# abhisrkckl/PulsePortraiture

Hardware: AMD Instinct MI355X
Metric: subint portrait fits/sec (phase+DM, 512ch×2048bin) at 1/2/4/8 MI355X (higher is better)
Workload: dtype f64

## Files before the change

### pulseportraiture_amd/csrc/ppf_wfft2.hpp

```cpp
#pragma once
#include "ppf_wfft.hpp"

namespace ppf {
namespace wf2 {

#define WF2_CUT() __builtin_amdgcn_sched_barrier(0)

constexpr int kN = 1024;
constexpr int kXS = 65;
constexpr int kXSlots = 16 * kXS;
constexpr int kSpSlots = 32;

struct Seeds {
    double2 w1;
    double2 v1;
};

__device__ __forceinline__ Seeds make_seeds(int lane) {
    Seeds s;
    double sn, cs;
    sincospi(-2.0 * (double)lane / 1024.0, &sn, &cs);
    s.w1 = cmk(cs, sn);
    sincospi(-2.0 * (double)(lane & 15) / 64.0, &sn, &cs);
    s.v1 = cmk(cs, sn);
// ... 47 lines not shown
        const double p = fma(-T[e], b.y, b.x), q = fma(T[e], b.x, b.y);
        u = cmk(fma(C[e], p, a.x), fma(C[e], q, a.y));
        v = cmk(fma(-C[e], p, a.x), fma(-C[e], q, a.y));
    }
}
template <int LEN, int I, int J>
__device__ __forceinline__ void dft16_bfly(double2 (&y)[16]) {
    if constexpr (J < LEN / 2) {
        bfly16<J * (16 / LEN)>(y[I + J], y[I + J + LEN / 2]);
        dft16_bfly<LEN, I, J + 1>(y);
    }
}
template <int LEN, int I>
__device__ __forceinline__ void dft16_group(double2 (&y)[16]) {
    if constexpr (I < 16) {
        dft16_bfly<LEN, I, 0>(y);
        dft16_group<LEN, I + LEN>(y);
    }
}
__device__ __forceinline__ void dft16(double2 (&x)[16]) {
    double2 y[16];
    wfft::dft_perm<16, 0>(x, y);
    dft16_group<2, 0>(y);
    dft16_group<4, 0>(y);
    dft16_group<8, 0>(y);
    dft16_group<16, 0>(y);
#pragma unroll
    for (int i = 0; i < 16; ++i) x[i] = y[i];
}

__device__ __forceinline__ void opaque(double2 &v) {
    asm volatile("" : "+v"(v.x), "+v"(v.y));
}
__device__ __forceinline__ void fft1024(double2 (&x)[16], double2 *xb, int lane, const Seeds &sd0) {
    Seeds sd = sd0;
    opaque(sd.w1);
    opaque(sd.v1);
    dft16(x);
    {
        double2 wq = sd.w1;
        x[1] = cmul(x[1], wq);
#pragma unroll
        for (int k = 2; k < 16; ++k) {
            wq = cmul(wq, sd.w1);
            x[k] = cmul(x[k], wq);
        }
    }
    WF2_CUT();
#pragma unroll
    for (int r = 0; r < 8; ++r) pswap<true>(x[r], x[r + 8]);
#pragma unroll
    for (int r = 0; r < 16; ++r)
        if ((r & 4) == 0) pswap<false>(x[r], x[r + 4]);
    const double2 v2 = cmul(sd.v1, sd.v1);
#pragma unroll
    for (int a = 0; a < 4; ++a) {
        double2 t[4] = {x[a], x[a + 4], x[a + 8], x[a + 12]};
        wfft::dft<4>(t);
        x[a] = t[0];
        x[a + 4] = cmul(t[1], sd.v1);
        x[a + 8] = cmulc(t[2], v2);
        x[a + 12] = cmulc(t[3], sd.v1);
    }
    WF2_CUT();
    const int llo = lane & 15, k1hi = lane >> 4;
    const int lb0 = kXS * llo + 4 * k1hi;
    const int lb1 = kXS * ((16 - llo) & 15) - 4 * k1hi + 32;
    const int lb8 = lb1 + (k1hi == 0 ? 0 : 32);
#pragma unroll
    for (int a = 0; a < 4; ++a) {
        xb[lb0 + a] = x[a];
        xb[lb0 + a + 16] = x[a + 4];
        if (a == 0) xb[lb8] = x[8];
        else xb[lb1 + 32 - a] = x[a + 8];
        xb[lb1 + 16 - a] = x[a + 12];
    }
    wfft::wave_sync();
#pragma unroll
    for (int r = 0; r < 16; ++r) x[r] = xb[lane + kXS * r];
    wfft::wave_sync();
    dft16(x);
}

__device__ __forceinline__ int lane_kappa(int lane) {
    return lane < 32 ? lane : (lane == 32 ? 32 : 96 - lane);
}
__device__ __forceinline__ int out_index(int lane, int m) {
    const int kap = lane_kappa(lane);
    return lane < 32 ? kap + 64 * m : kap + 64 * (15 - m);
}

__device__ __forceinline__ int pair_k0(int lane) {
    return lane == 32 ? 32 : (lane & 31) + (lane >= 32 ? 512 : 0);
}
__device__ __forceinline__ void pairs(double2 (&x)[16], double2 *sp, int lane, double2 &zm) {
    const bool special = (lane & 31) == 0;
    if (special) {
        const int b = (lane >> 5) * 16;
#pragma unroll
        for (int m = 0; m < 16; ++m) sp[b + m] = x[m];
    }
#pragma unroll
    for (int i = 0; i < 8; ++i) pswap<true>(x[i], x[i + 8]);
    wfft::wave_sync();
    if (special) {
        const bool l0 = lane == 0;
#pragma unroll
        for (int i = 0; i < 8; ++i) {
            x[i] = sp[l0 ? i : 31 - i];
            x[i + 8] = sp[l0 ? ((16 - i) & 15) : 16 + i];
        }
        if (l0) zm = sp[8];
    }
    wfft::wave_sync();
}

}
}
```

### pulseportraiture_amd/csrc/ppf_xspec.hip

```cpp
#include <cstdlib>
#include <cstring>
#include <type_traits>

#include "ppf_internal.hpp"
#include "ppf_state.hpp"
#include "ppf_wfft.hpp"
#include "ppf_wfft2.hpp"

namespace ppf {

constexpr int kXW = 8;
template <int LOG2N>
__host__ __device__ constexpr int xsw() { return LOG2N == 10 ? 4 : 8; }
typedef double f64x4 __attribute__((ext_vector_type(4)));
typedef float vf2 __attribute__((ext_vector_type(2)));
typedef double vd2 __attribute__((ext_vector_type(2)));
typedef float vf4 __attribute__((ext_vector_type(4)));
#define SCHED_CUT() __builtin_amdgcn_sched_barrier(0)

__device__ __forceinline__ void block_map(int xcd_swizzle, int nblk, int &s, int &cb, int nsub = 0) {
    if (xcd_swizzle == 2) {
        const int per = nblk / 8, x = blockIdx.x % 8, r = blockIdx.x / 8;
        cb = x * per + r / nsub;
        s = r % nsub;
// ... 514 lines not shown
            const double u = (double)(k - N / 2) * ih;
            const double v = u * u, v2 = v * v, v4 = v2 * v2, v8 = v4 * v4;
            const double bv = ((bj & 1) ? v : 1.0) * ((bj & 2) ? v2 : 1.0) * ((bj & 4) ? v4 : 1.0) *
                              ((bj & 8) ? v8 : 1.0);
            d0 = __builtin_amdgcn_mfma_f64_16x16x4f64(abase[2 * se], bv, d0, 0, 0, 0);
            d1 = __builtin_amdgcn_mfma_f64_16x16x4f64(abase[2 * so], bv, d1, 0, 0, 0);
        }
        XP(4);
        const int om = (tid >> 1) & 31, ori = tid & 1;
        double val = 0.0;
        if (om == 0) val = reinterpret_cast<const double *>(buf + SIDE)[ori];
        const double ie = reinterpret_cast<const double *>(buf + SIDE2)[0];
        __syncthreads();
        {
            double *sc = reinterpret_cast<double *>(buf);
#pragma unroll
            for (int rr = 0; rr < 4; ++rr) {
                sc[rr * 64 + lane] = d0[rr];
                sc[256 + rr * 64 + lane] = d1[rr];
            }
        }
        __syncthreads();
        {
            const int row = 2 * wave + ori;
            const int idx = (om & 1) * 256 + (row >> 2) * 64 + ((row & 3) << 4) + (om >> 1);
#pragma unroll
            for (int w2 = 0; w2 < XW; ++w2) val += reinterpret_cast<const double *>(lds + w2 * SLW)[idx];
            unsigned mo = (unsigned)(om * 2 + ori);
            asm volatile("" : "+v"(mo));
            if (live) mom[(int64_t)n * kMoments * 2 + mo] = val * ie;
        }
        __syncthreads();
        XP(5);
    }
    XP_DONE();
}

__global__ void k_btab(int N, double *Bt) {
    const int i = blockIdx.x * blockDim.x + threadIdx.x;
    if (i >= N / 2 * 16) return;
    const int k = i >> 4, j = i & 15;
    const double u = (double)(k - N / 2) * (2.0 / (double)N);
    const double v = u * u, v2 = v * v, v4 = v2 * v2, v8 = v4 * v4;
    Bt[i] = ((j & 1) ? v : 1.0) * ((j & 2) ? v2 : 1.0) * ((j & 4) ? v4 : 1.0) * ((j & 8) ? v8 : 1.0);
}

__global__ void k_model_pow(const double2 *Mft, int nrows, int nharm, double *out) {
    const int lane = threadIdx.x & 63;
    const int row = blockIdx.x * (blockDim.x >> 6) + (threadIdx.x >> 6);
    if (row >= nrows) return;
    const double2 *M = Mft + (int64_t)row * nharm;
    double acc = 0.0;
    for (int k = lane + 1; k < nharm; k += 64) acc += cabs2(M[k]);
    acc = wave_sum(acc);
    if (lane == 0) out[row] = acc;
}

__global__ __launch_bounds__(256) void k_model_sum(const double2 *Mft, int nchan, int nharm,
                                                   int nmodel, double2 *out) {
    __shared__ double2 part[16][17];
    const int kl = threadIdx.x & 15, grp = threadIdx.x >> 4;
    const int k = blockIdx.x * 16 + kl;
    const int m = blockIdx.y;
    const int per = (nchan + 15) / 16;
    const int n0 = grp * per, n1 = min(nchan, n0 + per);
    double2 acc = cmk(0.0, 0.0);
    if (k < nharm) {
        const double2 *M = Mft + (int64_t)m * nchan * nharm + k;
#pragma unroll 8
        for (int n = n0; n < n1; ++n) acc = cadd(acc, M[(int64_t)n * nharm]);
    }
    part[grp][kl] = acc;
    __syncthreads();
    if (grp == 0 && k < nharm) {
        double2 t = part[0][kl];
        for (int g = 1; g < 16; ++g) t = cadd(t, part[g][kl]);
        out[(int64_t)m * nharm + k] = t;
    }
}

constexpr int kX2W = 4;
constexpr int kX2SL = wf2::kXSlots + wf2::kSpSlots;
constexpr int kX2IE = 1041;
__device__ __forceinline__ int x2slot(int k) { return k + (k >> 6); }

template <int DT, bool GS, bool TL>
__device__ __forceinline__ void xspec_w2_block(const XspecArgs &a, const int s, const int cb) {
    constexpr int N = 1024, NH = N + 1;
    constexpr bool GR = TL;
    constexpr bool LT = GR && GS;
    constexpr int MD = 4;
    using RowT = typename std::conditional<DT == 0, vf2, vd2>::type;
    extern __shared__ __attribute__((aligned(16))) double2 lds[];
    const int lane0 = threadIdx.x & 63;
    const int wave = __builtin_amdgcn_readfirstlane(threadIdx.x >> 6);
    double2 *buf = lds + wave * kX2SL;

    const int cbase = cb * a.cb, cend = min(a.nchan, cbase + a.cb);
    const int nround = (cend - cbase + kX2W - 1) / kX2W;
    const RowT *rows = reinterpret_cast<const RowT *>(a.data);
    RowT zr[16];
    auto fetch = [&](int n) {
        const RowT *src = rows + ((int64_t)s * a.nchan + n) * N;
#pragma unroll
        for (int q = 0; q < 16; ++q) zr[q] = __builtin_nontemporal_load(src + lane0 + 64 * q);
    };
    auto fetch_c = [&](int m) { fetch(m < cend ? m : cend - 1); };
    auto rows_ready = [&]() {
#pragma unroll
        for (int q = 0; q < 16; ++q) asm volatile("" ::"v"(zr[q].x), "v"(zr[q].y));
    };
    int n = cbase + wave;
    if constexpr (TL) fetch_c(n);
    const int cls = a.cls[s];
    const int mi = a.model_index ? a.model_index[s] : 0;
    const int xsl = a.xslot ? a.xslot[s] : s;
    double g_Dg = 0.0, g_nrm2 = 0.0, g_w2e2 = 0.0;
    if constexpr (GS) {
        g_Dg = readfirst_d(a.rec[(int64_t)s * kRecN + kRecDg]);
        g_nrm2 = readfirst_d(a.rec[(int64_t)s * kRecN + kRecNuRefM2]);
    }
    if (a.needx && !(cls & kClsNeedX)) return;
    if (((cls & kClsTile) != 0) != TL) return;
    const bool gon = GS && (cls & kClsGflag) != 0;
    const uint8_t *mask = a.mask ? a.mask + (int64_t)s * a.nchan : nullptr;
    const int nl = cbase + lane0;
    const bool lin = nl < cend;
    const int nlc = lin ? nl : cend - 1;
    const int64_t scn = (int64_t)s * a.nchan + nlc;
    const int nkw = (cbase & ~63) + lane0;
    int ld_kc = a.KC ? a.KC[(int64_t)mi * a.nchan + (nkw < a.nchan ? nkw : a.nchan - 1)] : 0;
    int ld_mask = mask ? mask[nlc] : 1;
    double ld_mpow = a.Mpow[(int64_t)mi * a.nchan + nlc];
    double ld_err = a.errs ? a.errs[scn] : 0.0;
    double ld_wn = 0.0, ld_f = 1.0;
    if constexpr (GS) {
        ld_wn = a.guess_weights[scn];
        ld_f = a.freqs[scn];
    }
    const double sqrtN = sqrt((double)N);
    const wf2::Seeds sd = wf2::make_seeds(lane0);
    double2 wA0, wstep;
    {
        double sn, cs;
        sincospi(-(double)wf2::pair_k0(lane0) / (double)N, &sn, &cs);
        wA0 = cmk(cs, sn);
        sincospi(-64.0 / (double)N, &sn, &cs);
        wstep = cmk(cs, sn);
    }
    asm volatile("" : "+v"(ld_kc), "+v"(ld_mask), "+v"(ld_mpow), "+v"(ld_err), "+v"(ld_wn), "+v"(ld_f));
    double2 *Xs = a.X + (int64_t)xsl * a.xnh * a.nchan;
    int kw = NH;
    if (a.KC) kw = (int)wave_max(nkw < a.nchan ? (double)ld_kc : 1.0);
    auto store_tiles = [&](int n, const double2 *b, double ie2, bool ok) {
        const int kwp = (kw + kXTile - 1) & ~(kXTile - 1);
        double2 *Xn = Xs + (int64_t)n * kXTile + (lane0 & (kXTile - 1));
#pragma unroll 1
        for (int h = lane0; h < kwp; h += 64) {
            const double2 v = (ok && h < kw) ? cscale(b[x2slot(h)], ie2) : cmk(0.0, 0.0);
            __builtin_nontemporal_store(vd2{v.x, v.y},
                                        reinterpret_cast<vd2 *>(Xn + (int64_t)(h >> 3) * a.nchan * kXTile));
        }
    };
    const int mlane = (lin && ld_mask) ? 1 : 0;
    auto usable = [&](int n) {
        return n < cend && __builtin_amdgcn_readlane(mlane, n - cbase) != 0;
    };
    constexpr int NL = 64 * guess_npl(10);
    double2 *gacc = lds + kX2W * kX2SL;
    if constexpr (GS && !GR) {
        if (gon) {
            for (int t = threadIdx.x; t < NL; t += 64 * kX2W) gacc[t] = cmk(0.0, 0.0);
            __syncthreads();
        }
    }
    double2 gr[8];
#pragma unroll
    for (int i = 0; i < 8; ++i) gr[i] = cmk(0.0, 0.0);
    const double ch_mpow = lin ? ld_mpow : 0.0;
    const double ch_err = (a.errs && lin) ? ld_err : 0.0;
    double ch_wn = 0.0, ch_dg = 0.0;
    if (GS && gon && lin) {
        ch_wn = ld_wn;
        ch_dg = g_Dg * (1.0 / (ld_f * ld_f) - g_nrm2);
    }
    double2 ch_e1 = cmk(1.0, 0.0);
    if constexpr (GR) {
        if (GS && gon) ch_e1 = cexp2pi(ch_dg);
    }
    double2 *ltab = lds + kX2W * kX2SL;
    if constexpr (LT) {
        if (wave == 0) {
            ltab[lane0] = sd.w1;
            ltab[64 + lane0] = sd.v1;
            ltab[128 + lane0] = wA0;
            ltab[192 + lane0] = ch_e1;
        }
        __syncthreads();
    }
    if constexpr (!TL) fetch_c(n);
    rows_ready();
    XP_INIT();
    for (int r = 0; r < nround; ++r, n += kX2W) {
        const bool live = usable(n);
        if (n < cend && !live && lane0 < 4) a.chan[((int64_t)s * a.nchan + n) * 4 + lane0] = 0.0;
        double2 x[16];
#pragma unroll
        for (int q = 0; q < 16; ++q) {
            x[q] = cmk((double)zr[q].x, (double)zr[q].y);
            asm volatile("" : "+v"(x[q].x), "+v"(x[q].y));
        }
        int lane = lane0;
        asm volatile("" : "+v"(lane));
        const bool lo = lane <= 32;
        const int kA = wf2::pair_k0(lane);
        const int hl0 = lo ? kA : N - kA, hstep = lo ? 64 : -64;
        const double2 *Mrow = a.Mft + ((int64_t)mi * a.nchan + (n < cend ? n : cend - 1)) * NH;
        double2 Mq[MD > 0 ? MD : 1];
        auto mpre = [&]() {
#pragma unroll
            for (int i = 0; i < MD; ++i) Mq[i] = Mrow[(unsigned)(hl0 + hstep * i)];
        };
        SCHED_CUT();
        fetch_c(n + kX2W);
        if (live) {
            const int64_t crow = (int64_t)s * a.nchan + n;
            const int rr = n - cbase;
            XP(0);
            if constexpr (LT) {
                wf2::Seeds sdl;
                sdl.w1 = ltab[lane];
                sdl.v1 = ltab[64 + lane];
                wf2::fft1024(x, buf, lane, sdl);
            } else {
                wf2::fft1024(x, buf, lane, sd);
            }
            XP(1);
            SCHED_CUT();
            mpre();
            double2 zm = cmk(0.0, 0.0);
            wf2::pairs(x, buf + wf2::kXSlots, lane, zm);
            XP(2);
            double2 El = cmk(0.0, 0.0), Est = El;
            if constexpr (GR) {
                if (GS && gon) {
                    const double2 b1 = LT ? ltab[192 + rr] : cmk(readlane_d(ch_e1.x, rr), readlane_d(ch_e1.y, rr));
                    const double2 b2 = cmul(b1, b1), b4 = cmul(b2, b2), b8 = cmul(b4, b4);
                    const double2 b16 = cmul(b8, b8), b32 = cmul(b16, b16), b64 = cmul(b32, b32);
                    const int m = lane == 32 ? 32 : (lane & 31);
                    double2 pw = (m & 1) ? b1 : cmk(1.0, 0.0);
                    if (m & 2) pw = cmul(pw, b2);
                    if (m & 4) pw = cmul(pw, b4);
                    if (m & 8) pw = cmul(pw, b8);
                    if (m & 16) pw = cmul(pw, b16);
                    if (m & 32) pw = b32;
                    double2 E1 = pw;
                    if (!lo) {
                        const double2 b128 = cmul(b64, b64), b256 = cmul(b128, b128);
                        E1 = cmulc(cmul(b256, b256), pw);
                    }
                    El = cscale(E1, readlane_d(ch_wn, rr));
                    Est = lo ? b64 : cconj(b64);
                }
            } else if (GS && gon) {
                const double dg = readlane_d(ch_dg, rr);
                const double2 E1 = cexp2pi((double)hl0 * dg);
                El = cscale(E1, readlane_d(ch_wn, rr));
                Est = cmk(readlane_d(E1.x, 1), readlane_d(E1.y, 1));
#pragma unroll
                for (int q = 0; q < 6; ++q) Est = cmul(Est, Est);
                if (!lo) Est = cconj(Est);
            }
            const double sg = lo ? 1.0 : -1.0;
            const int hcut = N - a.kc;
            double pn = 0.0, pd = 0.0;
            double2 w = LT ? ltab[128 + lane] : wA0;
#pragma unroll
            for (int i = 0; i < 8; ++i) {
                const double2 zk = x[i], zn = x[i + 8];
                const double ex = zk.x + zn.x, ey = zk.y - zn.y;
                const double ox = zk.x - zn.x, oy = zk.y + zn.y;
                const double wox = fma(w.x, ox, -w.y * oy), woy = fma(w.x, oy, w.y * ox);
                w = cmul(w, wstep);
                const double ux = fma(sg, woy, ex), uy = fma(-sg, wox, ey);
                const double vx = fma(-sg, woy, ex), vy = fma(sg, wox, ey);
                const double2 Dl = cmk(ux, sg * uy);
                const double ph = fma(vx, vx, vy * vy), pl = fma(ux, ux, uy * uy);
                const int hl = hl0 + hstep * i;
                if (hl <= hcut) pn += ph;
                if (i == 0) pd += lane == 0 ? ph : pl + ph;
                else pd += pl + ph;
                double2 Ml;
                if constexpr (MD > 0) {
                    Ml = Mq[i % MD];
                    if (i + MD < 8) Mq[i % MD] = Mrow[(unsigned)(hl + hstep * MD)];
                } else {
                    Ml = Mrow[(unsigned)hl];
                }
                if (hl < kw) buf[x2slot(hl)] = cmulc(Dl, Ml);
                if (GS && gon) {
                    if constexpr (GR) gr[i] = cadd(gr[i], cmul(Dl, El));
                    else if (hl >= 1 && hl < NL) buf[x2slot(N - hl)] = cmul(Dl, El);
                    El = cmul(El, Est);
                } else if (kw > N / 2) {
                    const int hh = N - hl;
                    if (hh < kw) buf[x2slot(hh)] = cmulc(cmk(vx, -sg * vy), Mrow[(unsigned)hh]);
                }
            }
            XP(3);
            if (lane == 0) {
                buf[x2slot(0)] = cmk(0.0, 0.0);
                const double2 Dm = cmk(2.0 * zm.x, -2.0 * zm.y);
                const double p = cabs2(Dm);
                if (N / 2 >= a.kc) pn += p;
                pd += p;
                if (N / 2 < kw) buf[x2slot(N / 2)] = cmulc(Dm, Mrow[N / 2]);
            }
            pn *= 0.25;
            pd *= 0.25;
            pn = wave_sum(pn);
            pd = wave_sum(pd);
            double errs_FT;
            if (a.errs) errs_FT = readlane_d(ch_err, rr) * sqrtN;
            else errs_FT = sqrt(pn / (double)(NH - a.kc) / (double)(2 * N)) * sqrtN;
            const double inv_e2 = 1.0 / (errs_FT * errs_FT);
            if (GS && gon) {
                const double wn = readlane_d(ch_wn, rr);
                g_w2e2 += wn * wn * errs_FT * errs_FT;
            }
            const double mpow = readlane_d(ch_mpow, rr);
            if (lane == 0) {
                if constexpr (!TL) reinterpret_cast<double *>(buf + kX2IE)[0] = 0.5 * inv_e2;
                double *chan = a.chan + crow * 4;
                chan[0] = errs_FT;
                chan[1] = inv_e2;
                chan[2] = pd * inv_e2;
                chan[3] = mpow * inv_e2;
            }
            if constexpr (TL) {
                rows_ready();
                XP(4);
                wfft::wave_sync();
                store_tiles(n, buf, 0.5 * inv_e2, true);
                wfft::wave_sync();
                XP(5);
            }
        } else if constexpr (TL) {
            rows_ready();
            if (n < cend) store_tiles(n, buf, 0.0, false);
        }
        if constexpr (GR) continue;
        if (TL && !(GS && gon)) continue;
        if constexpr (!TL) {
            rows_ready();
            XP(4);
        }
        __syncthreads();
        XP(5);
        if constexpr (!TL) {
            const int c = threadIdx.x % kX2W, n0 = cbase + r * kX2W;
            const int nc = n0 + c;
            if (nc < cend) {
                const bool ok = !mask || mask[nc];
                const double2 *b = lds + c * kX2SL;
                const double ie2 = ok ? reinterpret_cast<const double *>(b + kX2IE)[0] : 0.0;
                for (int k = threadIdx.x / kX2W; k < kw; k += 64) {
                    const double2 v = ok ? cscale(b[x2slot(k)], ie2) : cmk(0.0, 0.0);
                    __builtin_nontemporal_store(vd2{v.x, v.y}, reinterpret_cast<vd2 *>(Xs + (int64_t)k * a.nchan + nc));
                }
            }
        }
        if (GS && gon) {
            for (int t = threadIdx.x; t < NL; t += 64 * kX2W) {
                if (t == 0) continue;
                double2 acc = gacc[t];
#pragma unroll
                for (int w2 = 0; w2 < kX2W; ++w2)
                    if (usable(cbase + r * kX2W + w2)) acc = cadd(acc, lds[w2 * kX2SL + x2slot(N - t)]);
                gacc[t] = acc;
            }
        }
        __syncthreads();
        XP(6);
    }
    {
        const int lane = lane0;
        (void)lane;
        XP_DONE();
    }
    if constexpr (GS) {
        if (gon) {
            double2 *gp = a.gpart + ((int64_t)s * a.nblk + cb) * NL;
            if constexpr (!GR)
                for (int t = threadIdx.x; t < NL; t += 64 * kX2W) gp[t] = cscale(gacc[t], 0.5);
            const double gwl = mlane ? ch_wn : 0.0;
            const double wsum = wave_sum(gwl), cnt = wave_sum(mlane ? 1.0 : 0.0);
            if constexpr (GR) {
                const bool lo = lane0 <= 32;
                const int kA = wf2::pair_k0(lane0);
                const int hl0 = lo ? kA : N - kA, hstep = lo ? 64 : -64;
#pragma unroll
                for (int i = 0; i < 8; ++i) {
                    const int hl = hl0 + hstep * i;
                    if (hl >= 1 && hl < NL) buf[hl] = gr[i];
                }
            }
            if (lane0 == 0) reinterpret_cast<double *>(buf)[0] = g_w2e2;
            __syncthreads();
            if constexpr (GR) {
                for (int t = threadIdx.x; t < NL; t += 64 * kX2W) {
                    double2 acc = cmk(0.0, 0.0);
                    if (t > 0) {
                        acc = lds[t];
#pragma unroll
                        for (int w2 = 1; w2 < kX2W; ++w2) acc = cadd(acc, lds[w2 * kX2SL + t]);
                    }
                    gp[t] = cscale(acc, 0.5);
                }
            }
            if (threadIdx.x == 0) {
                double acc = 0.0;
                for (int w2 = 0; w2 < kX2W; ++w2) acc += reinterpret_cast<const double *>(lds + w2 * kX2SL)[0];
                double *o = a.gw + ((int64_t)s * a.nblk + cb) * 3;
                o[0] = wsum;
                o[1] = cnt;
                o[2] = acc;
            }
        }
    }
}

template <int DT, bool GS, bool TL>
__global__ __launch_bounds__(64 * kX2W) __attribute__((amdgpu_waves_per_eu(2)))
void k_xspec_w2(XspecArgs a) {
    int s, cb;
    block_map(a.xcd_swizzle, a.nblk, s, cb, a.nsub);
    xspec_w2_block<DT, GS, TL>(a, s, cb);
}

constexpr int kX2ListGrid = 512;
template <int DT, bool GS>
__global__ __launch_bounds__(64 * kX2W) __attribute__((amdgpu_waves_per_eu(2)))
void k_xspec_w2_list(XspecArgs a) {
    const int64_t items = (int64_t)*a.nlist * a.nblk;
    for (int64_t it = blockIdx.x; it < items; it += gridDim.x) {
        xspec_w2_block<DT, GS, false>(a, a.list[it / a.nblk], (int)(it % a.nblk));
        __syncthreads();
    }
}

constexpr int kWmW = 4;
constexpr int kWmMaxN = 1024;

__device__ __forceinline__ int mod_small(int j, int L, float invL) {
    const int q = (int)((float)j * invL);
    int k = j - q * L;
    k += k < 0 ? L : 0;
    k -= k >= L ? L : 0;
    return k;
}

template <int R, int NMAX>
__device__ __forceinline__ void wmr_stage(double2 *buf, int N, int L, const double2 *tw, int lane) {
    constexpr int QM = (NMAX / R + 63) / 64;
    const int nb = N / R, ts = N / (R * L);
    const float invL = 1.0f / (float)L;
    double2 x[QM][R];
#pragma unroll
    for (int q = 0; q < QM; ++q) {
        const int j = lane + 64 * q;
        if (j < nb) {
            const int k = mod_small(j, L, invL);
#pragma unroll
            for (int r = 0; r < R; ++r) x[q][r] = buf[j + r * nb];
#pragma unroll
            for (int r = 1; r < R; ++r) x[q][r] = cmul(x[q][r], tw[r * k * ts]);
            dft_small<R>(x[q], false);
        }
    }
    wfft::wave_sync();
#pragma unroll
    for (int q = 0; q < QM; ++q) {
        const int j = lane + 64 * q;
        if (j < nb) {
            const int k = mod_small(j, L, invL);
            const int o = (j - k) * R + k;
#pragma unroll
            for (int r = 0; r < R; ++r) buf[o + r * L] = x[q][r];
        }
    }
    wfft::wave_sync();
}

template <int NMAX>
__device__ __forceinline__ void wmr_stage_g(double2 *buf, int N, int L, int R, const double2 *tw, int lane) {
    double2 y[NMAX / 64];
    gr_stage_read4<NMAX / 64>(buf, N, L, R, tw, false, lane, 64, y);
    wfft::wave_sync();
    gr_stage_write<NMAX / 64>(buf, N, lane, 64, y);
    wfft::wave_sync();
}

template <int DT, int NMAX, bool ODD>
__global__ __launch_bounds__(64 * kWmW) __attribute__((amdgpu_waves_per_eu(NMAX <= 512 ? 3 : 2)))
void k_xspec_wm(XspecArgs a) {
    const int N = a.nbin >> 1, NH = N + 1;
    const int NF = ODD ? a.nbin : N;
    const int SL = ODD ? NF : N + 2, IE = N + 1;
    extern __shared__ __attribute__((aligned(16))) double2 lds[];
    const int lane = threadIdx.x & 63, wave = threadIdx.x >> 6;
    double2 *buf = lds + wave * SL;
    double2 *twl = lds + kWmW * SL;
    int s, cb;
    block_map(a.xcd_swizzle, a.nblk, s, cb, a.nsub);
    if (a.needx && !a.needx[s]) return;
    for (int i = threadIdx.x; i < NF; i += 64 * kWmW) twl[i] = a.T[i];
    __syncthreads();
    const int cbase = cb * a.cb, cend = min(a.nchan, cbase + a.cb);
    const int nround = (a.cb + kWmW - 1) / kWmW;
    const int mi = a.model_index ? a.model_index[s] : 0;
    const uint8_t *mask = a.mask ? a.mask + (int64_t)s * a.nchan : nullptr;
    const double sqrtN = sqrt((double)a.nbin / 2.0);
    double2 *Xs = a.X + (int64_t)(a.xslot ? a.xslot[s] : s) * NH * a.nchan;
    int kw = NH;
    if (a.KC) {
        const int nn = (cbase & ~63) + lane;
        kw = (int)wave_max(nn < a.nchan ? (double)a.KC[(int64_t)mi * a.nchan + nn] : 1.0);
    }
    const int mlane = (cbase + lane < cend && (!mask || mask[cbase + lane])) ? 1 : 0;
// ... 234 lines not shown
        }
        __syncthreads();
        {
            const int c = threadIdx.x % RW, nc = cbase + r * RW + c;
            if (nc < cend) {
                const bool ok = !mask || mask[nc];
                const double2 *b = lds + (c % kWmW) * SL;
                const int o0 = c < kWmW ? 0 : NF, st = c < kWmW ? 1 : -1;
                const double ie2 = ok ? b[o0].x : 0.0;
                for (int k = threadIdx.x / RW; k < kw; k += 64 * kWmW / RW)
                    st_stream(Xs + (int64_t)k * a.nchan + nc, (ok && k) ? cscale(b[o0 + st * k], ie2) : cmk(0.0, 0.0));
            }
        }
        __syncthreads();
    }
}

bool xspec_wm_supported(int nbin) {
    if (nbin & 1) return nbin >= 33 && nbin < kWmMaxN;
    const int N = nbin / 2;
    return !is_pow2(N) && N <= kWmMaxN && fft_len_supported(N);
}

#define PPF_WM_LAUNCH(NM, ODD)                                                           \
    do {                                                                                 \
        if (a.dtype == 0) hipLaunchKernelGGL((k_xspec_wm<0, NM, ODD>), g, b, lds, st, a); \
        else hipLaunchKernelGGL((k_xspec_wm<1, NM, ODD>), g, b, lds, st, a);              \
    } while (0)

static bool use_xspec_wo() {
    static const bool on = [] {
        const char *e = getenv("PPF_XSPEC_WO");
        return e ? atoi(e) != 0 : true;
    }();
    return on;
}

hipError_t launch_xspec_wm(const XspecArgs &a, hipStream_t st) {
    const bool odd = a.nbin & 1;
    const int NF = rfft_len(a.nbin);
    if (odd && use_xspec_wo()) {
        const size_t lds = ((size_t)kWmW * (NF + 1) + NF) * sizeof(double2);
        dim3 g((unsigned)((int64_t)a.nsub * a.nblk)), b(64 * kWmW);
        if (NF <= 512) {
            if (a.dtype == 0) hipLaunchKernelGGL((k_xspec_wo<0, 512>), g, b, lds, st, a);
            else hipLaunchKernelGGL((k_xspec_wo<1, 512>), g, b, lds, st, a);
        } else {
            if (a.dtype == 0) hipLaunchKernelGGL((k_xspec_wo<0, 1024>), g, b, lds, st, a);
            else hipLaunchKernelGGL((k_xspec_wo<1, 1024>), g, b, lds, st, a);
        }
        return hipGetLastError();
    }
    const size_t lds = ((size_t)kWmW * (odd ? NF : NF + 2) + NF) * sizeof(double2);
    dim3 g((unsigned)((int64_t)a.nsub * a.nblk)), b(64 * kWmW);
    if (NF <= 512) {
        if (odd) PPF_WM_LAUNCH(512, true);
        else PPF_WM_LAUNCH(512, false);
    } else {
        if (odd) PPF_WM_LAUNCH(1024, true);
        else PPF_WM_LAUNCH(1024, false);
    }
    return hipGetLastError();
}

static bool use_xspec2() {
    static const bool on = [] {
        const char *e = getenv("PPF_XSPEC2");
        return e ? atoi(e) != 0 : true;
    }();
    return on;
}
bool xspec_tiled(int log2N) {
    static const bool on = [] {
        const char *e = getenv("PPF_XTILE");
        return e ? atoi(e) != 0 : true;
    }();
    return on && log2N == 10 && use_xspec2();
}

template <int L2, int DT>
static void launch_w(const XspecArgs &a, hipStream_t st) {
    if constexpr (L2 == 10) {
        if (use_xspec2()) {
            const size_t lds = (size_t)kX2W * kX2SL * sizeof(double2);
            dim3 g((unsigned)((int64_t)a.nsub * a.nblk)), b(64 * kX2W);
            if (a.xtile) {
                if (a.gflag)
                    hipLaunchKernelGGL((k_xspec_w2<DT, true, true>), g, b,
                                       lds + (size_t)256 * sizeof(double2), st, a);
                else hipLaunchKernelGGL((k_xspec_w2<DT, false, true>), g, b, lds, st, a);
            }
            const dim3 gh = a.list ? dim3(kX2ListGrid) : g;
            if (a.gflag) {
                const size_t ldg = lds + (size_t)guess_slots(10) * sizeof(double2);
                if (a.list) hipLaunchKernelGGL((k_xspec_w2_list<DT, true>), gh, b, ldg, st, a);
                else hipLaunchKernelGGL((k_xspec_w2<DT, true, false>), gh, b, ldg, st, a);
            } else {
                if (a.list) hipLaunchKernelGGL((k_xspec_w2_list<DT, false>), gh, b, lds, st, a);
                else hipLaunchKernelGGL((k_xspec_w2<DT, false, false>), gh, b, lds, st, a);
            }
            return;
        }
    }
    const size_t lds = ((size_t)xsw<L2>() * xspec_slw<L2>() + tw_slots<L2>()) * sizeof(double2);
    dim3 g((unsigned)((int64_t)a.nsub * a.nblk)), b(64 * xsw<L2>());
    if (a.gflag && L2 == 10)
        hipLaunchKernelGGL((k_xspec_w<L2, DT, L2 == 10>), g, b,
                           lds + (size_t)guess_slots(L2) * sizeof(double2), st, a);
    else hipLaunchKernelGGL((k_xspec_w<L2, DT, false>), g, b, lds, st, a);
}

int xspec_own_cb(int log2N) { return (log2N == 10 && use_xspec2()) ? 64 : 0; }

bool xspec_wave_supported(int log2N, int cb) {
    return log2N >= 7 && log2N <= 10 && cb % xsw<7>() == 0 && cb % xsw<10>() == 0 && cb % kXW == 0;
}

hipError_t launch_xspec_wave(const XspecArgs &a, hipStream_t st) {
    switch (a.log2N * 2 + a.dtype) {
        case 14: launch_w<7, 0>(a, st); break;
        case 15: launch_w<7, 1>(a, st); break;
        case 16: launch_w<8, 0>(a, st); break;
        case 17: launch_w<8, 1>(a, st); break;
        case 18: launch_w<9, 0>(a, st); break;
        case 19: launch_w<9, 1>(a, st); break;
        case 20: launch_w<10, 0>(a, st); break;
        case 21: launch_w<10, 1>(a, st); break;
        default: return hipErrorInvalidValue;
    }
    return hipGetLastError();
}

constexpr int kNoiseW = 4;
template <int LOG2N, int DT>
__global__ __launch_bounds__(64 * kNoiseW) void k_noise_w(NoiseArgs a, int64_t nrows) {
    using P = wfft::Plan<LOG2N>;
    constexpr int N = P::N, R = P::R, NP = N / 128;
    constexpr int SL = wfft::buf_slots<LOG2N>();
    using RowT = typename std::conditional<DT == 0, vf2, vd2>::type;
    extern __shared__ __attribute__((aligned(16))) double2 lds[];
    const int lane = threadIdx.x & 63, wave = threadIdx.x >> 6;
    double2 *buf = lds + wave * SL;
    double2 *tw = lds + kNoiseW * SL;
    for (int i = threadIdx.x; i < tw_slots<LOG2N>(); i += 64 * kNoiseW) tw[i] = a.T[i];
    __syncthreads();
    const double2 w_seed = a.T2[lane], w_step = a.T2[64];
    const RowT *rows = reinterpret_cast<const RowT *>(a.in);
    const int64_t nw = (int64_t)gridDim.x * kNoiseW;
    int64_t row = (int64_t)blockIdx.x * kNoiseW + wave;
    RowT zr[R];
    auto fetch = [&](int64_t rr) {
        const RowT *src = rows + rr * N;
#pragma unroll
        for (int q = 0; q < R; ++q) zr[q] = src[lane + 64 * q];
    };
    if (row < nrows) fetch(row);
    for (; row < nrows; row += nw) {
        double2 x[R];
#pragma unroll
        for (int q = 0; q < R; ++q) x[q] = cmk((double)zr[q].x, (double)zr[q].y);
        if (row + nw < nrows) fetch(row + nw);
        wfft::fft_row<LOG2N>(x, buf, tw, lane);
        double pn = 0.0;
        double2 w = w_seed;
#pragma unroll
        for (int i = 0; i < NP; ++i) {
            const int klo = lane + 64 * i, khi = N - klo;
            double2 Dlo, Dhi;
            rfft_pair<LOG2N>(buf, klo, w, Dlo, Dhi);
            w = cmul(w, w_step);
            if (klo >= a.kc) pn += cabs2(Dlo);
            if (khi >= a.kc) pn += cabs2(Dhi);
// ... 275 lines not shown
```

Baseline: 335,000.

## Reorder pair lanes, add direct register-to-global tile stores, move per-channel scalars to LDS

Changes the pair-exchange layout so every lane walks harmonics with a positive stride of 64 (x[i] paired with x[15-i]). When the kept width is at most half the spectrum, products go straight from registers to global memory with nontemporal stores instead of being staged through LDS tiles. Per-channel scalars (mpow, err, wn, dg) move from readlane broadcasts into a small LDS table, and the Mft prefetch depth and guess-accumulator count are tuned per dtype and path. This adds LDS footprint, and the wider store pattern risks less coalesced global writes.

```diff
diff --git a/pulseportraiture_amd/csrc/ppf_wfft2.hpp b/pulseportraiture_amd/csrc/ppf_wfft2.hpp
--- a/pulseportraiture_amd/csrc/ppf_wfft2.hpp
+++ b/pulseportraiture_amd/csrc/ppf_wfft2.hpp
@@ -162,7 +162,7 @@
 }
 
 __device__ __forceinline__ int pair_k0(int lane) {
-    return lane == 32 ? 32 : (lane & 31) + (lane >= 32 ? 512 : 0);
+    return lane < 32 ? lane : kN - lane_kappa(lane);
 }
 __device__ __forceinline__ void pairs(double2 (&x)[16], double2 *sp, int lane, double2 &zm) {
     const bool special = (lane & 31) == 0;
@@ -172,14 +172,15 @@
         for (int m = 0; m < 16; ++m) sp[b + m] = x[m];
     }
 #pragma unroll
-    for (int i = 0; i < 8; ++i) pswap<true>(x[i], x[i + 8]);
+    for (int i = 0; i < 8; ++i) pswap<true>(x[i], x[15 - i]);
     wfft::wave_sync();
     if (special) {
         const bool l0 = lane == 0;
 #pragma unroll
         for (int i = 0; i < 8; ++i) {
-            x[i] = sp[l0 ? i : 31 - i];
-            x[i + 8] = sp[l0 ? ((16 - i) & 15) : 16 + i];
+            const double2 v = sp[l0 ? ((16 - i) & 15) : 16 + i];
+            if (l0) x[15 - i] = v;
+            else x[i] = v;
         }
         if (l0) zm = sp[8];
     }
diff --git a/pulseportraiture_amd/csrc/ppf_xspec.hip b/pulseportraiture_amd/csrc/ppf_xspec.hip
--- a/pulseportraiture_amd/csrc/ppf_xspec.hip
+++ b/pulseportraiture_amd/csrc/ppf_xspec.hip
@@ -620,14 +620,16 @@
 constexpr int kX2W = 4;
 constexpr int kX2SL = wf2::kXSlots + wf2::kSpSlots;
 constexpr int kX2IE = 1041;
+constexpr int kX2LT = 5, kX2LTG = 6;
 __device__ __forceinline__ int x2slot(int k) { return k + (k >> 6); }
 
-template <int DT, bool GS, bool TL>
+template <int DT, bool GS, bool TL, bool LS = false>
 __device__ __forceinline__ void xspec_w2_block(const XspecArgs &a, const int s, const int cb) {
     constexpr int N = 1024, NH = N + 1;
     constexpr bool GR = TL;
     constexpr bool LT = GR && GS;
-    constexpr int MD = 4;
+    constexpr bool DR = TL && DT == 0;
+    constexpr int MD = LS ? (DT == 0 ? 2 : 1) : (DT == 0 ? 4 : ((TL && GS) ? 1 : 2));
     using RowT = typename std::conditional<DT == 0, vf2, vd2>::type;
     extern __shared__ __attribute__((aligned(16))) double2 lds[];
     const int lane0 = threadIdx.x & 63;
@@ -689,7 +691,20 @@
     asm volatile("" : "+v"(ld_kc), "+v"(ld_mask), "+v"(ld_mpow), "+v"(ld_err), "+v"(ld_wn), "+v"(ld_f));
     double2 *Xs = a.X + (int64_t)xsl * a.xnh * a.nchan;
     int kw = NH;
-    if (a.KC) kw = (int)wave_max(nkw < a.nchan ? (double)ld_kc : 1.0);
+    if (a.KC) kw = __builtin_amdgcn_readfirstlane((int)wave_max(nkw < a.nchan ? (double)ld_kc : 1.0));
+    auto store_direct = [&](int n, int lane, int kw, const double2 (&P)[8], double ie2, bool ok) {
+        const int kwp = (kw + kXTile - 1) & ~(kXTile - 1);
+        const int off = wf2::lane_kappa(lane);
+        double2 *Xn = Xs + (int64_t)n * kXTile + (off & (kXTile - 1)) + (int64_t)(off >> 3) * a.nchan * kXTile;
+        const int64_t sst = (int64_t)(64 / kXTile) * a.nchan * kXTile;
+#pragma unroll
+        for (int i = 0; i < 8; ++i) {
+            if (64 * i >= kwp) break;
+            const int h = 64 * i + off;
+            const double2 v = (ok && h >= 1 && h < kw) ? cscale(P[i], ie2) : cmk(0.0, 0.0);
+            if (h < kwp) __builtin_nontemporal_store(vd2{v.x, v.y}, reinterpret_cast<vd2 *>(Xn + i * sst));
+        }
+    };
     auto store_tiles = [&](int n, const double2 *b, double ie2, bool ok) {
         const int kwp = (kw + kXTile - 1) & ~(kXTile - 1);
         double2 *Xn = Xs + (int64_t)n * kXTile + (lane0 & (kXTile - 1));
@@ -712,9 +727,10 @@
             __syncthreads();
         }
     }
-    double2 gr[8];
-#pragma unroll
-    for (int i = 0; i < 8; ++i) gr[i] = cmk(0.0, 0.0);
+    constexpr int NS = NL / 64;
+    double2 gr[NS];
+#pragma unroll
+    for (int i = 0; i < NS; ++i) gr[i] = cmk(0.0, 0.0);
     const double ch_mpow = lin ? ld_mpow : 0.0;
     const double ch_err = (a.errs && lin) ? ld_err : 0.0;
     double ch_wn = 0.0, ch_dg = 0.0;
@@ -726,16 +742,18 @@
     if constexpr (GR) {
         if (GS && gon) ch_e1 = cexp2pi(ch_dg);
     }
-    double2 *ltab = lds + kX2W * kX2SL;
-    if constexpr (LT) {
-        if (wave == 0) {
-            ltab[lane0] = sd.w1;
-            ltab[64 + lane0] = sd.v1;
-            ltab[128 + lane0] = wA0;
-            ltab[192 + lane0] = ch_e1;
-        }
-        __syncthreads();
-    }
+    double2 *ltab = lds + kX2W * kX2SL + ((GS && !GR) ? NL : 0);
+    if (wave == 0) {
+        ltab[lane0] = sd.w1;
+        ltab[64 + lane0] = sd.v1;
+        ltab[128 + lane0] = wA0;
+        ltab[192 + lane0] = cmk(ch_mpow, ch_err);
+        ltab[256 + lane0] = cmk(ch_wn, ch_dg);
+        if constexpr (LT) {
+            ltab[320 + lane0] = ch_e1;
+        }
+    }
+    __syncthreads();
     if constexpr (!TL) fetch_c(n);
     rows_ready();
     XP_INIT();
@@ -750,14 +768,16 @@
         }
         int lane = lane0;
         asm volatile("" : "+v"(lane));
-        const bool lo = lane <= 32;
-        const int kA = wf2::pair_k0(lane);
-        const int hl0 = lo ? kA : N - kA, hstep = lo ? 64 : -64;
+        int kwr = __builtin_amdgcn_readfirstlane(kw), hcut = __builtin_amdgcn_readfirstlane(N - a.kc);
+        asm volatile("" : "+s"(kwr), "+s"(hcut));
+        const bool direct = DR && kwr <= N / 2;
+        const bool lo = lane < 32;
+        const int hl0 = wf2::lane_kappa(lane);
         const double2 *Mrow = a.Mft + ((int64_t)mi * a.nchan + (n < cend ? n : cend - 1)) * NH;
         double2 Mq[MD > 0 ? MD : 1];
         auto mpre = [&]() {
 #pragma unroll
-            for (int i = 0; i < MD; ++i) Mq[i] = Mrow[(unsigned)(hl0 + hstep * i)];
+            for (int i = 0; i < MD; ++i) Mq[i] = Mrow[(unsigned)(hl0 + 64 * i)];
         };
         SCHED_CUT();
         fetch_c(n + kX2W);
@@ -765,13 +785,11 @@
             const int64_t crow = (int64_t)s * a.nchan + n;
             const int rr = n - cbase;
             XP(0);
-            if constexpr (LT) {
+            {
                 wf2::Seeds sdl;
                 sdl.w1 = ltab[lane];
                 sdl.v1 = ltab[64 + lane];
                 wf2::fft1024(x, buf, lane, sdl);
-            } else {
-                wf2::fft1024(x, buf, lane, sd);
             }
             XP(1);
             SCHED_CUT();
@@ -780,93 +798,93 @@
             wf2::pairs(x, buf + wf2::kXSlots, lane, zm);
             XP(2);
             double2 El = cmk(0.0, 0.0), Est = El;
-            if constexpr (GR) {
-                if (GS && gon) {
-                    const double2 b1 = LT ? ltab[192 + rr] : cmk(readlane_d(ch_e1.x, rr), readlane_d(ch_e1.y, rr));
+            if constexpr (LT) {
+                if (gon) {
+                    const double2 b1 = ltab[320 + rr];
                     const double2 b2 = cmul(b1, b1), b4 = cmul(b2, b2), b8 = cmul(b4, b4);
-                    const double2 b16 = cmul(b8, b8), b32 = cmul(b16, b16), b64 = cmul(b32, b32);
-                    const int m = lane == 32 ? 32 : (lane & 31);
+                    const double2 b16 = cmul(b8, b8), b32 = cmul(b16, b16);
+                    const int m = lane & 31;
                     double2 pw = (m & 1) ? b1 : cmk(1.0, 0.0);
                     if (m & 2) pw = cmul(pw, b2);
                     if (m & 4) pw = cmul(pw, b4);
                     if (m & 8) pw = cmul(pw, b8);
                     if (m & 16) pw = cmul(pw, b16);
-                    if (m & 32) pw = b32;
+                    Est = cmul(b32, b32);
                     double2 E1 = pw;
-                    if (!lo) {
-                        const double2 b128 = cmul(b64, b64), b256 = cmul(b128, b128);
-                        E1 = cmulc(cmul(b256, b256), pw);
-                    }
-                    El = cscale(E1, readlane_d(ch_wn, rr));
-                    Est = lo ? b64 : cconj(b64);
+                    if (!lo) E1 = m == 0 ? b32 : cmulc(Est, pw);
+                    El = cscale(E1, ltab[256 + rr].x);
                 }
             } else if (GS && gon) {
-                const double dg = readlane_d(ch_dg, rr);
-                const double2 E1 = cexp2pi((double)hl0 * dg);
-                El = cscale(E1, readlane_d(ch_wn, rr));
+                const double2 wd = ltab[256 + rr];
+                const double2 E1 = cexp2pi((double)hl0 * wd.y);
+                El = cscale(E1, wd.x);
                 Est = cmk(readlane_d(E1.x, 1), readlane_d(E1.y, 1));
 #pragma unroll
                 for (int q = 0; q < 6; ++q) Est = cmul(Est, Est);
-                if (!lo) Est = cconj(Est);
             }
             const double sg = lo ? 1.0 : -1.0;
-            const int hcut = N - a.kc;
             double pn = 0.0, pd = 0.0;
-            double2 w = LT ? ltab[128 + lane] : wA0;
+            double2 w = ltab[128 + lane];
+            const double2 wst = cmk(wstep.x, sg * wstep.y);
+            double2 P[8];
 #pragma unroll
             for (int i = 0; i < 8; ++i) {
-                const double2 zk = x[i], zn = x[i + 8];
+                const double2 zk = x[i], zn = x[15 - i];
                 const double ex = zk.x + zn.x, ey = zk.y - zn.y;
                 const double ox = zk.x - zn.x, oy = zk.y + zn.y;
                 const double wox = fma(w.x, ox, -w.y * oy), woy = fma(w.x, oy, w.y * ox);
-                w = cmul(w, wstep);
+                if (i + 1 < 8) w = cmul(w, wst);
                 const double ux = fma(sg, woy, ex), uy = fma(-sg, wox, ey);
                 const double vx = fma(-sg, woy, ex), vy = fma(sg, wox, ey);
                 const double2 Dl = cmk(ux, sg * uy);
                 const double ph = fma(vx, vx, vy * vy), pl = fma(ux, ux, uy * uy);
-                const int hl = hl0 + hstep * i;
+                const int hl = hl0 + 64 * i;
                 if (hl <= hcut) pn += ph;
                 if (i == 0) pd += lane == 0 ? ph : pl + ph;
                 else pd += pl + ph;
                 double2 Ml;
                 if constexpr (MD > 0) {
                     Ml = Mq[i % MD];
-                    if (i + MD < 8) Mq[i % MD] = Mrow[(unsigned)(hl + hstep * MD)];
+                    if (i + MD < 8) Mq[i % MD] = Mrow[(unsigned)(hl + 64 * MD)];
                 } else {
                     Ml = Mrow[(unsigned)hl];
                 }
-                if (hl < kw) buf[x2slot(hl)] = cmulc(Dl, Ml);
+                P[i] = cmulc(Dl, Ml);
+                if (!direct && hl < kwr) buf[x2slot(hl)] = P[i];
                 if (GS && gon) {
-                    if constexpr (GR) gr[i] = cadd(gr[i], cmul(Dl, El));
-                    else if (hl >= 1 && hl < NL) buf[x2slot(N - hl)] = cmul(Dl, El);
-                    El = cmul(El, Est);
-                } else if (kw > N / 2) {
+                    if (i < NS) {
+                        if constexpr (GR) gr[i] = cadd(gr[i], cmul(Dl, El));
+                        else if (hl >= 1) buf[x2slot(N - hl)] = cmul(Dl, El);
+                        if (i + 1 < NS) El = cmul(El, Est);
+                    }
+                } else if (kwr > N / 2) {
                     const int hh = N - hl;
-                    if (hh < kw) buf[x2slot(hh)] = cmulc(cmk(vx, -sg * vy), Mrow[(unsigned)hh]);
+                    if (hh < kwr) buf[x2slot(hh)] = cmulc(cmk(vx, -sg * vy), Mrow[(unsigned)hh]);
                 }
             }
             XP(3);
             if (lane == 0) {
-                buf[x2slot(0)] = cmk(0.0, 0.0);
+                if (!direct) buf[x2slot(0)] = cmk(0.0, 0.0);
                 const double2 Dm = cmk(2.0 * zm.x, -2.0 * zm.y);
                 const double p = cabs2(Dm);
                 if (N / 2 >= a.kc) pn += p;
                 pd += p;
-                if (N / 2 < kw) buf[x2slot(N / 2)] = cmulc(Dm, Mrow[N / 2]);
+                if (N / 2 < kwr) buf[x2slot(N / 2)] = cmulc(Dm, Mrow[N / 2]);
             }
             pn *= 0.25;
             pd *= 0.25;
             pn = wave_sum(pn);
             pd = wave_sum(pd);
             double errs_FT;
-            if (a.errs) errs_FT = readlane_d(ch_err, rr) * sqrtN;
+            const double2 me = ltab[192 + rr];
+            if (a.errs) errs_FT = me.y * sqrtN;
             else errs_FT = sqrt(pn / (double)(NH - a.kc) / (double)(2 * N)) * sqrtN;
             const double inv_e2 = 1.0 / (errs_FT * errs_FT);
             if (GS && gon) {
-                const double wn = readlane_d(ch_wn, rr);
+                const double wn = ltab[256 + rr].x;
                 g_w2e2 += wn * wn * errs_FT * errs_FT;
             }
-            const double mpow = readlane_d(ch_mpow, rr);
+            const double mpow = me.x;
             if (lane == 0) {
                 if constexpr (!TL) reinterpret_cast<double *>(buf + kX2IE)[0] = 0.5 * inv_e2;
                 double *chan = a.chan + crow * 4;
@@ -878,14 +896,22 @@
             if constexpr (TL) {
                 rows_ready();
                 XP(4);
-                wfft::wave_sync();
-                store_tiles(n, buf, 0.5 * inv_e2, true);
-                wfft::wave_sync();
+                if (direct) {
+                    store_direct(n, lane, kwr, P, 0.5 * inv_e2, true);
+                } else {
+                    wfft::wave_sync();
+                    store_tiles(n, buf, 0.5 * inv_e2, true);
+                    wfft::wave_sync();
+                }
                 XP(5);
             }
         } else if constexpr (TL) {
             rows_ready();
-            if (n < cend) store_tiles(n, buf, 0.0, false);
+            if (n < cend) {
+                const double2 Pz[8] = {};
+                if (direct) store_direct(n, lane, kwr, Pz, 0.0, false);
+                else store_tiles(n, buf, 0.0, false);
+            }
         }
         if constexpr (GR) continue;
         if (TL && !(GS && gon)) continue;
@@ -931,16 +957,14 @@
             double2 *gp = a.gpart + ((int64_t)s * a.nblk + cb) * NL;
             if constexpr (!GR)
                 for (int t = threadIdx.x; t < NL; t += 64 * kX2W) gp[t] = cscale(gacc[t], 0.5);
-            const double gwl = mlane ? ch_wn : 0.0;
+            const double gwl = mlane ? ltab[256 + lane0].x : 0.0;
             const double wsum = wave_sum(gwl), cnt = wave_sum(mlane ? 1.0 : 0.0);
             if constexpr (GR) {
-                const bool lo = lane0 <= 32;
-                const int kA = wf2::pair_k0(lane0);
-                const int hl0 = lo ? kA : N - kA, hstep = lo ? 64 : -64;
-#pragma unroll
-                for (int i = 0; i < 8; ++i) {
-                    const int hl = hl0 + hstep * i;
-                    if (hl >= 1 && hl < NL) buf[hl] = gr[i];
+                const int hl0 = wf2::lane_kappa(lane0);
+#pragma unroll
+                for (int i = 0; i < NS; ++i) {
+                    const int hl = hl0 + 64 * i;
+                    if (hl >= 1) buf[hl] = gr[i];
                 }
             }
             if (lane0 == 0) reinterpret_cast<double *>(buf)[0] = g_w2e2;
@@ -982,7 +1006,7 @@
 void k_xspec_w2_list(XspecArgs a) {
     const int64_t items = (int64_t)*a.nlist * a.nblk;
     for (int64_t it = blockIdx.x; it < items; it += gridDim.x) {
-        xspec_w2_block<DT, GS, false>(a, a.list[it / a.nblk], (int)(it % a.nblk));
+        xspec_w2_block<DT, GS, false, true>(a, a.list[it / a.nblk], (int)(it % a.nblk));
         __syncthreads();
     }
 }
@@ -1383,12 +1407,12 @@
 static void launch_w(const XspecArgs &a, hipStream_t st) {
     if constexpr (L2 == 10) {
         if (use_xspec2()) {
-            const size_t lds = (size_t)kX2W * kX2SL * sizeof(double2);
+            const size_t lds = ((size_t)kX2W * kX2SL + kX2LT * 64) * sizeof(double2);
             dim3 g((unsigned)((int64_t)a.nsub * a.nblk)), b(64 * kX2W);
             if (a.xtile) {
                 if (a.gflag)
                     hipLaunchKernelGGL((k_xspec_w2<DT, true, true>), g, b,
-                                       lds + (size_t)256 * sizeof(double2), st, a);
+                                       lds + (size_t)(kX2LTG - kX2LT) * 64 * sizeof(double2), st, a);
                 else hipLaunchKernelGGL((k_xspec_w2<DT, false, true>), g, b, lds, st, a);
             }
             const dim3 gh = a.list ? dim3(kX2ListGrid) : g;
```

Measured after the change: 338,300, median of 6. No clear change (+1.0%).

## Remap FFT pair lanes so each band stays in registers and store tiles directly

Applied to the files above, without the earlier changes.

Reorders the real-FFT pair unpacking so that register slot i of every lane holds harmonic band i (kappa + 64*i) instead of a mirrored descending layout. With that layout, the tiled path keeps cross-spectrum values in registers and writes them straight to global memory with nontemporal stores when kw <= N/2. This skips the LDS staging buffer and the wave syncs around store_tiles. It also trims the guess-gradient accumulators to whole bands below NL and skips the full pair computation for bands above the cutoffs. A constexpr static_assert checks the new pairing, but the rewritten index mapping and the GS twiddle/power recomputation carry correctness risk.

```diff
diff --git a/pulseportraiture_amd/csrc/ppf_wfft2.hpp b/pulseportraiture_amd/csrc/ppf_wfft2.hpp
--- a/pulseportraiture_amd/csrc/ppf_wfft2.hpp
+++ b/pulseportraiture_amd/csrc/ppf_wfft2.hpp
@@ -153,17 +153,47 @@
     dft16(x);
 }
 
-__device__ __forceinline__ int lane_kappa(int lane) {
+constexpr __host__ __device__ int lane_kappa(int lane) {
     return lane < 32 ? lane : (lane == 32 ? 32 : 96 - lane);
 }
-__device__ __forceinline__ int out_index(int lane, int m) {
-    const int kap = lane_kappa(lane);
-    return lane < 32 ? kap + 64 * m : kap + 64 * (15 - m);
-}
-
-__device__ __forceinline__ int pair_k0(int lane) {
-    return lane == 32 ? 32 : (lane & 31) + (lane >= 32 ? 512 : 0);
-}
+constexpr __host__ __device__ int out_index(int lane, int m) {
+    return lane < 32 ? lane_kappa(lane) + 64 * m : lane_kappa(lane) + 64 * (15 - m);
+}
+
+constexpr __host__ __device__ bool pair_lo(int lane) { return lane < 32; }
+constexpr __host__ __device__ int pair_hl(int lane, int i) { return 64 * i + lane_kappa(lane); }
+constexpr __host__ __device__ int pair_k(int lane, int i) {
+    return pair_lo(lane) ? pair_hl(lane, i) : kN - pair_hl(lane, i);
+}
+constexpr __host__ __device__ int pair_src_a(int lane, int i) {
+    return lane == 0    ? out_index(0, i)
+           : lane == 32 ? out_index(32, i)
+           : lane < 32  ? out_index(lane, i)
+                        : out_index(lane - 32, 15 - i);
+}
+constexpr __host__ __device__ int pair_src_b(int lane, int i) {
+    return lane == 0    ? out_index(0, (16 - i) & 15)
+           : lane == 32 ? out_index(32, 15 - i)
+           : lane < 32  ? out_index(lane + 32, i)
+                        : out_index(lane, 15 - i);
+}
+constexpr __host__ __device__ bool pairs_ok() {
+    for (int i = 0; i < 8; ++i) {
+        bool seen[64] = {};
+        for (int lane = 0; lane < 64; ++lane) {
+            const int hl = pair_hl(lane, i);
+            const int za = pair_src_a(lane, i), zb = pair_src_b(lane, i);
+            if (hl < 64 * i || hl > 64 * i + 63 || seen[hl - 64 * i]) return false;
+            seen[hl - 64 * i] = true;
+            if ((za + zb) % kN != 0) return false;
+            if ((pair_lo(lane) ? za : zb) != hl) return false;
+            if (pair_k(lane, i) % kN != za) return false;
+        }
+    }
+    return out_index(0, 8) == kN / 2;
+}
+static_assert(pairs_ok(), "wf2::pairs: slot i of every lane is one pair (hl, N - hl) of band i");
+
 __device__ __forceinline__ void pairs(double2 (&x)[16], double2 *sp, int lane, double2 &zm) {
     const bool special = (lane & 31) == 0;
     if (special) {
@@ -172,14 +202,14 @@
         for (int m = 0; m < 16; ++m) sp[b + m] = x[m];
     }
 #pragma unroll
-    for (int i = 0; i < 8; ++i) pswap<true>(x[i], x[i + 8]);
+    for (int i = 0; i < 8; ++i) pswap<true>(x[i], x[15 - i]);
     wfft::wave_sync();
     if (special) {
         const bool l0 = lane == 0;
 #pragma unroll
         for (int i = 0; i < 8; ++i) {
-            x[i] = sp[l0 ? i : 31 - i];
-            x[i + 8] = sp[l0 ? ((16 - i) & 15) : 16 + i];
+            x[i] = sp[l0 ? i : 16 + i];
+            x[15 - i] = sp[l0 ? ((16 - i) & 15) : 31 - i];
         }
         if (l0) zm = sp[8];
     }
diff --git a/pulseportraiture_amd/csrc/ppf_xspec.hip b/pulseportraiture_amd/csrc/ppf_xspec.hip
--- a/pulseportraiture_amd/csrc/ppf_xspec.hip
+++ b/pulseportraiture_amd/csrc/ppf_xspec.hip
@@ -681,7 +681,7 @@
     double2 wA0, wstep;
     {
         double sn, cs;
-        sincospi(-(double)wf2::pair_k0(lane0) / (double)N, &sn, &cs);
+        sincospi(-(double)wf2::pair_k(lane0, 0) / (double)N, &sn, &cs);
         wA0 = cmk(cs, sn);
         sincospi(-64.0 / (double)N, &sn, &cs);
         wstep = cmk(cs, sn);
@@ -690,6 +690,8 @@
     double2 *Xs = a.X + (int64_t)xsl * a.xnh * a.nchan;
     int kw = NH;
     if (a.KC) kw = (int)wave_max(nkw < a.nchan ? (double)ld_kc : 1.0);
+    constexpr bool RX = TL;
+    const bool rx = kw <= N / 2;
     auto store_tiles = [&](int n, const double2 *b, double ie2, bool ok) {
         const int kwp = (kw + kXTile - 1) & ~(kXTile - 1);
         double2 *Xn = Xs + (int64_t)n * kXTile + (lane0 & (kXTile - 1));
@@ -712,9 +714,11 @@
             __syncthreads();
         }
     }
-    double2 gr[8];
-#pragma unroll
-    for (int i = 0; i < 8; ++i) gr[i] = cmk(0.0, 0.0);
+    constexpr int NG = NL / 64;
+    static_assert(NL == 64 * NG && NG < 8, "whole bands of guess harmonics");
+    double2 gr[NG];
+#pragma unroll
+    for (int i = 0; i < NG; ++i) gr[i] = cmk(0.0, 0.0);
     const double ch_mpow = lin ? ld_mpow : 0.0;
     const double ch_err = (a.errs && lin) ? ld_err : 0.0;
     double ch_wn = 0.0, ch_dg = 0.0;
@@ -750,14 +754,13 @@
         }
         int lane = lane0;
         asm volatile("" : "+v"(lane));
-        const bool lo = lane <= 32;
-        const int kA = wf2::pair_k0(lane);
-        const int hl0 = lo ? kA : N - kA, hstep = lo ? 64 : -64;
+        const bool lo = wf2::pair_lo(lane);
+        const int kap = wf2::lane_kappa(lane);
         const double2 *Mrow = a.Mft + ((int64_t)mi * a.nchan + (n < cend ? n : cend - 1)) * NH;
         double2 Mq[MD > 0 ? MD : 1];
         auto mpre = [&]() {
 #pragma unroll
-            for (int i = 0; i < MD; ++i) Mq[i] = Mrow[(unsigned)(hl0 + hstep * i)];
+            for (int i = 0; i < MD; ++i) Mq[i] = Mrow[(unsigned)(kap + 64 * i)];
         };
         SCHED_CUT();
         fetch_c(n + kX2W);
@@ -784,70 +787,77 @@
                 if (GS && gon) {
                     const double2 b1 = LT ? ltab[192 + rr] : cmk(readlane_d(ch_e1.x, rr), readlane_d(ch_e1.y, rr));
                     const double2 b2 = cmul(b1, b1), b4 = cmul(b2, b2), b8 = cmul(b4, b4);
-                    const double2 b16 = cmul(b8, b8), b32 = cmul(b16, b16), b64 = cmul(b32, b32);
-                    const int m = lane == 32 ? 32 : (lane & 31);
-                    double2 pw = (m & 1) ? b1 : cmk(1.0, 0.0);
-                    if (m & 2) pw = cmul(pw, b2);
-                    if (m & 4) pw = cmul(pw, b4);
-                    if (m & 8) pw = cmul(pw, b8);
-                    if (m & 16) pw = cmul(pw, b16);
-                    if (m & 32) pw = b32;
-                    double2 E1 = pw;
-                    if (!lo) {
-                        const double2 b128 = cmul(b64, b64), b256 = cmul(b128, b128);
-                        E1 = cmulc(cmul(b256, b256), pw);
-                    }
-                    El = cscale(E1, readlane_d(ch_wn, rr));
-                    Est = lo ? b64 : cconj(b64);
+                    const double2 b16 = cmul(b8, b8), b32 = cmul(b16, b16);
+                    double2 pw = (kap & 1) ? b1 : cmk(1.0, 0.0);
+                    if (kap & 2) pw = cmul(pw, b2);
+                    if (kap & 4) pw = cmul(pw, b4);
+                    if (kap & 8) pw = cmul(pw, b8);
+                    if (kap & 16) pw = cmul(pw, b16);
+                    if (kap & 32) pw = cmul(pw, b32);
+                    El = cscale(pw, readlane_d(ch_wn, rr));
+                    Est = cmul(b32, b32);
                 }
             } else if (GS && gon) {
                 const double dg = readlane_d(ch_dg, rr);
-                const double2 E1 = cexp2pi((double)hl0 * dg);
+                const double2 E1 = cexp2pi((double)kap * dg);
                 El = cscale(E1, readlane_d(ch_wn, rr));
                 Est = cmk(readlane_d(E1.x, 1), readlane_d(E1.y, 1));
 #pragma unroll
                 for (int q = 0; q < 6; ++q) Est = cmul(Est, Est);
-                if (!lo) Est = cconj(Est);
             }
             const double sg = lo ? 1.0 : -1.0;
+            const double2 ws = cmk(wstep.x, sg * wstep.y);
             const int hcut = N - a.kc;
+            const bool gq = GS && gon;
             double pn = 0.0, pd = 0.0;
             double2 w = LT ? ltab[128 + lane] : wA0;
 #pragma unroll
             for (int i = 0; i < 8; ++i) {
-                const double2 zk = x[i], zn = x[i + 8];
+                const double2 zk = x[i], zn = x[15 - i];
+                if (i >= NG && !(64 * i < kw || 64 * i <= hcut)) {
+                    pd = fma(4.0, fma(zk.x, zk.x, zk.y * zk.y) + fma(zn.x, zn.x, zn.y * zn.y), pd);
+                    continue;
+                }
                 const double ex = zk.x + zn.x, ey = zk.y - zn.y;
                 const double ox = zk.x - zn.x, oy = zk.y + zn.y;
                 const double wox = fma(w.x, ox, -w.y * oy), woy = fma(w.x, oy, w.y * ox);
-                w = cmul(w, wstep);
+                if (i < 7) w = cmul(w, ws);
                 const double ux = fma(sg, woy, ex), uy = fma(-sg, wox, ey);
                 const double vx = fma(-sg, woy, ex), vy = fma(sg, wox, ey);
                 const double2 Dl = cmk(ux, sg * uy);
                 const double ph = fma(vx, vx, vy * vy), pl = fma(ux, ux, uy * uy);
-                const int hl = hl0 + hstep * i;
+                const int hl = kap + 64 * i;
                 if (hl <= hcut) pn += ph;
                 if (i == 0) pd += lane == 0 ? ph : pl + ph;
                 else pd += pl + ph;
                 double2 Ml;
                 if constexpr (MD > 0) {
                     Ml = Mq[i % MD];
-                    if (i + MD < 8) Mq[i % MD] = Mrow[(unsigned)(hl + hstep * MD)];
+                    if (i + MD < 8) Mq[i % MD] = Mrow[(unsigned)(hl + 64 * MD)];
                 } else {
                     Ml = Mrow[(unsigned)hl];
                 }
-                if (hl < kw) buf[x2slot(hl)] = cmulc(Dl, Ml);
-                if (GS && gon) {
-                    if constexpr (GR) gr[i] = cadd(gr[i], cmul(Dl, El));
-                    else if (hl >= 1 && hl < NL) buf[x2slot(N - hl)] = cmul(Dl, El);
-                    El = cmul(El, Est);
+                const double2 xv = cmulc(Dl, Ml);
+                if constexpr (RX) x[i] = xv;
+                else if (hl < kw) buf[x2slot(hl)] = xv;
+                if (gq) {
+                    if (i < NG) {
+                        if constexpr (GR) gr[i] = cadd(gr[i], cmul(Dl, El));
+                        else if (hl >= 1) buf[x2slot(N - hl)] = cmul(Dl, El);
+                        El = cmul(El, Est);
+                    }
                 } else if (kw > N / 2) {
+                    if (RX && hl < kw) buf[x2slot(hl)] = xv;
                     const int hh = N - hl;
                     if (hh < kw) buf[x2slot(hh)] = cmulc(cmk(vx, -sg * vy), Mrow[(unsigned)hh]);
                 }
             }
+            if (lane == 0) {
+                if constexpr (RX) x[0] = cmk(0.0, 0.0);
+                if (!(RX && rx)) buf[x2slot(0)] = cmk(0.0, 0.0);
+            }
             XP(3);
             if (lane == 0) {
-                buf[x2slot(0)] = cmk(0.0, 0.0);
                 const double2 Dm = cmk(2.0 * zm.x, -2.0 * zm.y);
                 const double p = cabs2(Dm);
                 if (N / 2 >= a.kc) pn += p;
@@ -878,9 +888,25 @@
             if constexpr (TL) {
                 rows_ready();
                 XP(4);
-                wfft::wave_sync();
-                store_tiles(n, buf, 0.5 * inv_e2, true);
-                wfft::wave_sync();
+                if (rx) {
+                    const double ie2 = 0.5 * inv_e2;
+                    const int kwp = (kw + kXTile - 1) & ~(kXTile - 1);
+                    double2 *Xn = Xs + (int64_t)n * kXTile + (kap & (kXTile - 1)) +
+                                  (int64_t)(kap >> 3) * a.nchan * kXTile;
+#pragma unroll
+                    for (int i = 0; i < 8; ++i) {
+                        if (64 * i >= kw) break;
+                        const int h = kap + 64 * i;
+                        const double2 v = h < kw ? cscale(x[i], ie2) : cmk(0.0, 0.0);
+                        if (h < kwp)
+                            __builtin_nontemporal_store(
+                                vd2{v.x, v.y}, reinterpret_cast<vd2 *>(Xn + (int64_t)(8 * i) * a.nchan * kXTile));
+                    }
+                } else {
+                    wfft::wave_sync();
+                    store_tiles(n, buf, 0.5 * inv_e2, true);
+                    wfft::wave_sync();
+                }
                 XP(5);
             }
         } else if constexpr (TL) {
@@ -934,13 +960,10 @@
             const double gwl = mlane ? ch_wn : 0.0;
             const double wsum = wave_sum(gwl), cnt = wave_sum(mlane ? 1.0 : 0.0);
             if constexpr (GR) {
-                const bool lo = lane0 <= 32;
-                const int kA = wf2::pair_k0(lane0);
-                const int hl0 = lo ? kA : N - kA, hstep = lo ? 64 : -64;
-#pragma unroll
-                for (int i = 0; i < 8; ++i) {
-                    const int hl = hl0 + hstep * i;
-                    if (hl >= 1 && hl < NL) buf[hl] = gr[i];
+#pragma unroll
+                for (int i = 0; i < NG; ++i) {
+                    const int hl = wf2::pair_hl(lane0, i);
+                    if (hl >= 1) buf[hl] = gr[i];
                 }
             }
             if (lane0 == 0) reinterpret_cast<double *>(buf)[0] = g_w2e2;
```

Result: faster. 334,200 before, 347,200 after, median of 6 (+3.9%).
